# PetarKirov/Chess2RT

Hardware: AMD Instinct MI355X
Metric: Mray/s (reference-equivalent rays per second: one primary ray per sample + one shadow ray per (hit, lit light), counted as the reference casts them; ms/frame in ms_per_step) (higher is better)
Workload: dtype f64; 1 GPU; lecture5.sdl 3840x2160, 5 tap(s)/pixel (AAEnabled as shipped: reference 5-tap AA), dof off; primary_rays_per_frame=41472000, full=False

## Files before the change

### chess2rt_amd/_abi.py

```python
import ctypes as C
import os

_HERE = os.path.dirname(os.path.abspath(__file__))
_VARIANT = os.environ.get("C2RT_LIB_VARIANT", "")
LIB_PATH = os.path.join(_HERE, "libc2rt%s.so" % ("_" + _VARIANT if _VARIANT else ""))

OK, ERR_INVALID_ARG, ERR_NO_DEVICE, ERR_HIP, ERR_UNSUPPORTED, ERR_LIMIT, ERR_NO_SCENE, ERR_CANCELLED, ERR_IO, ERR_PARSE = range(10)
GEOM_PLANE, GEOM_SPHERE, GEOM_CUBE, GEOM_CSG_UNION, GEOM_CSG_INTER, GEOM_CSG_DIFF = range(6)
SHADER_LAMBERT, SHADER_PHONG = 0, 1
TEX_CHECKER, TEX_PROCEDURE2, TEX_BITMAP = 0, 1, 2
LIGHT_POINT = 0
TAPS_1, TAPS_REF5, TAPS_4 = 1, 5, 4
ABI_VERSION = 1
MAX_CSG_DEPTH = 4
MAX_CSG_HITS = 8
MAX_BATCH_FRAMES = 256
MAX_RAYS = 1 << 28
MAX_HIT_LAYERS = 16
AA_THRESHOLD_REF = 0.1

_i32p = C.POINTER(C.c_int32)
_u32p = C.POINTER(C.c_uint32)
_u64p = C.POINTER(C.c_uint64)
_f32p = C.POINTER(C.c_float)
# ... 169 lines not shown
        ("pos", C.c_double * 3),
        ("yaw", C.c_double), ("pitch", C.c_double), ("roll", C.c_double), ("fov", C.c_double),
        ("focal_plane_dist", C.c_double), ("f_number", C.c_double), ("disc_multiplier", C.c_double),
        ("dof", C.c_uint32),
        ("num_samples", C.c_uint64),
        ("stereo_separation", C.c_double),
    ]


_SCENE_P = C.POINTER(SceneDesc)
_CAM_P = C.POINTER(CameraFrame)
_OPTS_P = C.POINTER(RenderOpts)
_POSE_P = C.POINTER(ScenePose)
_VP = C.c_void_p

C2RT_SYMBOLS = {
    "c2rt_init": (C.c_int, [C.c_int, C.POINTER(_VP)]),
    "c2rt_init_multi": (C.c_int, [C.c_int, C.POINTER(C.c_int), C.POINTER(_VP)]),
    "c2rt_device_count": (C.c_int, [_VP]),
    "c2rt_scene_generation": (C.c_uint64, [_VP]),
    "c2rt_get_csg_truncations": (C.c_int, [_VP, C.POINTER(C.c_uint64)]),
    "c2rt_get_exact_redos": (C.c_int, [_VP, C.POINTER(C.c_uint64)]),
    "c2rt_get_ground_bails": (C.c_int, [_VP, C.POINTER(C.c_uint64)]),
    "c2rt_destroy": (None, [_VP]),
    "c2rt_last_error": (C.c_char_p, [_VP]),
    "c2rt_status_string": (C.c_char_p, [C.c_int]),
    "c2rt_abi_version": (C.c_uint32, []),
    "c2rt_upload_scene": (C.c_int, [_VP, _SCENE_P]),
    "c2rt_update_scene": (C.c_int, [_VP, _POSE_P, _VP]),
    "c2rt_local_rows": (C.c_uint32, [_OPTS_P]),
    "c2rt_render_frame": (C.c_int, [_VP, _CAM_P, _OPTS_P, _VP, _VP]),
    "c2rt_render_frame_device": (C.c_int, [_VP, _CAM_P, _OPTS_P, _VP, _VP]),
    "c2rt_render_frames": (C.c_int, [_VP, _CAM_P, C.c_uint32, _OPTS_P, _VP, _VP]),
    "c2rt_render_frames_device": (C.c_int, [_VP, _CAM_P, C.c_uint32, _OPTS_P, _VP, _VP]),
    "c2rt_render_frames_posed": (C.c_int, [_VP, _CAM_P, _POSE_P, C.c_uint32, _OPTS_P, _VP, _VP]),
    "c2rt_render_frames_posed_device": (C.c_int, [_VP, _CAM_P, _POSE_P, C.c_uint32, _OPTS_P, _VP, _VP]),
    "c2rt_pin_host_buffer": (C.c_int, [_VP, _VP, C.c_size_t]),
    "c2rt_unpin_host_buffer": (C.c_int, [_VP, _VP]),
    "c2rt_get_ray_stats": (C.c_int, [_VP, C.POINTER(RayStats)]),
    "c2rt_render_pixel": (C.c_int, [_VP, _CAM_P, _OPTS_P, C.c_int, C.c_int, C.POINTER(TraceResult)]),
    "c2rt_trace_rays_device": (C.c_int, [_VP, _VP, C.c_uint64, _VP, _VP, _VP]),
    "c2rt_trace_rays": (C.c_int, [_VP, _VP, C.c_uint64, _VP, _VP]),
    "c2rt_test_visibility_device": (C.c_int, [_VP, _VP, C.c_uint64, _VP, _VP]),
    "c2rt_test_visibility": (C.c_int, [_VP, _VP, C.c_uint64, _VP]),
    "c2rt_render_hits_device": (C.c_int, [_VP, _CAM_P, _OPTS_P, C.POINTER(HitPlanes), _VP]),
    "c2rt_render_hits": (C.c_int, [_VP, _CAM_P, _OPTS_P, C.POINTER(HitPlanes)]),
# ... 88 lines not shown
```

### chess2rt_amd/api.py

```python
import ctypes as C

import numpy as np

from . import _abi
from ._abi import (CameraFrame, HitPlanes, HostCamera, HostSettings, Ray, RayHit, RayStats, RenderOpts, SceneDesc, ScenePose, Segment,
                   ShadePlanes, TraceResult)

RAY_HIT_DTYPE = np.dtype({
    "names": ["closest_node", "leaf_geom", "dist", "u", "v", "p", "normal"],
    "formats": [np.int32, np.int32, np.float64, np.float64, np.float64, (np.float64, 3), (np.float64, 3)],
    "offsets": [RayHit.closest_node.offset, RayHit.leaf_geom.offset, RayHit.dist.offset, RayHit.u.offset, RayHit.v.offset,
                RayHit.p.offset, RayHit.normal.offset],
    "itemsize": C.sizeof(RayHit),
})


HIT_PLANES = {"node": (np.int32, 1), "leaf": (np.int32, 1), "dist": (np.float64, 1), "uv": (np.float64, 2),
              "p": (np.float64, 3), "normal": (np.float64, 3), "rgb": (np.float32, 3)}


def _new_hit_planes(names, rows, width):
    names = tuple(names)
    for n in names:
        if n not in HIT_PLANES:
# ... 373 lines not shown
        self._check(self._lib.c2rt_render_frames_posed_adaptive_device(self._h, arr, parr, n, C.byref(opts), float(threshold),
                                                                       C.c_void_p(out_ptr or None), C.c_void_p(mask_ptr or None), C.c_void_p(stream)))

    def rayStats(self):
        s = RayStats()
        self._check(self._lib.c2rt_get_ray_stats(self._h, C.byref(s)))
        return int(s.primary_rays), int(s.shadow_rays)

    def csgTruncations(self):
        n = C.c_uint64()
        self._check(self._lib.c2rt_get_csg_truncations(self._h, C.byref(n)))
        return int(n.value)

    def exactRedos(self):
        n = C.c_uint64()
        self._check(self._lib.c2rt_get_exact_redos(self._h, C.byref(n)))
        return int(n.value)

    def groundBails(self):
        n = C.c_uint64()
        self._check(self._lib.c2rt_get_ground_bails(self._h, C.byref(n)))
        return int(n.value)

    def renderPixel(self, cam, opts, x, y):
        r = TraceResult()
        self._check(self._lib.c2rt_render_pixel(self._h, C.byref(cam), C.byref(opts), int(x), int(y), C.byref(r)))
        return r

    def traceRays(self, rays, hits=True, colors=True):
        rays = np.ascontiguousarray(rays, dtype=np.float64)
        if rays.ndim != 2 or rays.shape[1] != 6:
            raise ValueError("rays: expected shape (n, 6), got %r" % (rays.shape,))
        n = rays.shape[0]
        rec = np.empty(n, dtype=RAY_HIT_DTYPE) if hits else None
        rgb = np.empty((n, 3), dtype=np.float32) if colors else None
        self._check(self._lib.c2rt_trace_rays(self._h, rays.ctypes.data_as(C.c_void_p), n,
                                              rec.ctypes.data_as(C.c_void_p) if hits else None,
                                              rgb.ctypes.data_as(C.c_void_p) if colors else None))
        return rec, rgb

    def traceRaysDevice(self, rays_ptr, n, hits_ptr, rgb_ptr, stream=0):
        self._check(self._lib.c2rt_trace_rays_device(self._h, C.c_void_p(rays_ptr), int(n), C.c_void_p(hits_ptr or None),
                                                     C.c_void_p(rgb_ptr or None), C.c_void_p(stream)))

    def traceRayLayers(self, rays, max_layers, hits=True, colors=True):
        rays = np.ascontiguousarray(rays, dtype=np.float64)
# ... 225 lines not shown
```

### chess2rt_amd/csrc/c2rt_api.cpp

```cpp
#include <hip/hip_runtime.h>

#include <atomic>
#include <cmath>
#include <cstdint>
#include <cstdarg>
#include <cstdio>
#include <cstdlib>
#include <cstring>
#include <memory>
#include <string>
#include <utility>
#include <vector>

#include "c2rt_query.h"
#include "scene_plan.h"

using namespace c2rt;

constexpr int kMaxChunks = 16;

constexpr int kScratchSlots = 16;
struct FrameScratch {
    const void *key = nullptr;
    bool used = false;
// ... 479 lines not shown
    }
}

const char *c2rt_last_error(const c2rt_ctx *ctx) { return ctx ? ctx->err.c_str() : "null context"; }

int c2rt_init(int device, c2rt_ctx **out)
{
    if (!out) return C2RT_ERR_INVALID_ARG;
    *out = nullptr;
    int count = 0;
    if (hipGetDeviceCount(&count) != hipSuccess || count <= 0) return C2RT_ERR_NO_DEVICE;
    if (device >= count) return C2RT_ERR_NO_DEVICE;
    if (device < 0 && hipGetDevice(&device) != hipSuccess) return C2RT_ERR_NO_DEVICE;
    c2rt_ctx *ctx = new c2rt_ctx();
    ctx->device = device;
    *out = ctx;
    HIP_TRY(ctx, hipSetDevice(device));
    HIP_TRY(ctx, hipStreamCreateWithFlags(&ctx->stream, hipStreamNonBlocking));
    HIP_TRY(ctx, hipStreamCreateWithFlags(&ctx->copy_stream, hipStreamNonBlocking));
    for (int i = 0; i < kMaxChunks; ++i) HIP_TRY(ctx, hipEventCreateWithFlags(&ctx->chunk_done[i], hipEventDisableTiming));
    HIP_TRY(ctx, hipEventCreateWithFlags(&ctx->ev_ready, hipEventDisableTiming));
    HIP_TRY(ctx, hipEventCreateWithFlags(&ctx->ev_done, hipEventDisableTiming));
    HIP_TRY(ctx, hipEventCreateWithFlags(&ctx->ev_inflight, hipEventDisableTiming));
    HIP_TRY(ctx, hipMalloc(reinterpret_cast<void **>(&ctx->counters), 5 * sizeof(unsigned long long)));
    HIP_TRY(ctx, hipMemset(ctx->counters, 0, 5 * sizeof(unsigned long long)));
    HIP_TRY(ctx, hipMalloc(reinterpret_cast<void **>(&ctx->probe), sizeof(c2rt_trace_result)));
    uint8_t lut[4097];
    build_srgb_lut(lut);
    HIP_TRY(ctx, hipMalloc(reinterpret_cast<void **>(&ctx->srgb_lut), sizeof lut));
    HIP_TRY(ctx, hipMemcpy(ctx->srgb_lut, lut, sizeof lut, hipMemcpyHostToDevice));
    return C2RT_OK;
}

int c2rt_init_multi(int device_count_or_0, const int *device_ids, c2rt_ctx **out)
{
    if (!out) return C2RT_ERR_INVALID_ARG;
    *out = nullptr;
    int visible = 0;
    if (hipGetDeviceCount(&visible) != hipSuccess || visible <= 0) return C2RT_ERR_NO_DEVICE;
    if (device_count_or_0 < 0 || device_count_or_0 > 64) return C2RT_ERR_INVALID_ARG;
    const int n = device_count_or_0 == 0 ? visible : device_count_or_0;
    std::vector<int> ids(n);
    for (int i = 0; i < n; ++i) {
        ids[i] = (device_ids && device_count_or_0 > 0) ? device_ids[i] : i;
        if (ids[i] < 0 || ids[i] >= visible) return C2RT_ERR_NO_DEVICE;
    }
    c2rt_ctx *lead = nullptr;
    int st = c2rt_init(ids[0], &lead);
// ... 573 lines not shown
    }
    if (!ctx->peers.empty()) HIP_TRY(ctx, hipSetDevice(ctx->device));
    return C2RT_OK;
}

int c2rt_get_ground_bails(c2rt_ctx *ctx, uint64_t *out)
{
    if (!ctx || !out) return C2RT_ERR_INVALID_ARG;
    HIP_TRY(ctx, hipSetDevice(ctx->device));
    HIP_TRY(ctx, hipDeviceSynchronize());
    unsigned long long h = 0;
    HIP_TRY(ctx, hipMemcpy(&h, ctx->counters + 4, sizeof h, hipMemcpyDeviceToHost));
    *out = h;
    for (c2rt_ctx *c : ctx->peers) {
        HIP_TRY(ctx, hipSetDevice(c->device));
        HIP_TRY(ctx, hipDeviceSynchronize());
        HIP_TRY(ctx, hipMemcpy(&h, c->counters + 4, sizeof h, hipMemcpyDeviceToHost));
        *out += h;
    }
    if (!ctx->peers.empty()) HIP_TRY(ctx, hipSetDevice(ctx->device));
    return C2RT_OK;
}

int c2rt_render_pixel(c2rt_ctx *ctx, const c2rt_camera_frame *cam, const c2rt_render_opts *opts, int x, int y,
                      c2rt_trace_result *out)
{
    int st = check_frame_args(ctx, cam, opts);
    if (st != C2RT_OK) return st;
    if (!out) return fail(ctx, C2RT_ERR_INVALID_ARG, "null output");
    HIP_TRY(ctx, hipSetDevice(ctx->device));
    RenderParams p;
    frame_params(ctx, cam, opts, p);
    p.n_cull = 0;
    p.ground_fast = 0;
    p.ground_certain_cq = 0;
    p.n_cull_lights = 0;
    p.csg_cap = (uint32_t)kCsgFullCap(C2RT_MAX_CSG_DEPTH);
    p.probe_x = x;
    p.probe_y = y;
    p.probe_out = ctx->probe;
    HIP_TRY(ctx, hipMemsetAsync(ctx->probe, 0, sizeof(c2rt_trace_result), ctx->stream));
    const int e = launch_probe(p, variant_of(ctx->plan, cam), ctx->stream);
    if (e != 0) return fail(ctx, C2RT_ERR_HIP, "probe kernel launch: %s", hipGetErrorString((hipError_t)e));
    HIP_TRY(ctx, hipMemcpyAsync(out, ctx->probe, sizeof *out, hipMemcpyDeviceToHost, ctx->stream));
    HIP_TRY(ctx, hipStreamSynchronize(ctx->stream));
    return C2RT_OK;
// ... 765 lines not shown
```

### chess2rt_amd/csrc/c2rt_shade_planes.hip

```cpp
#define C2RT_TRACE_EXACT_ONLY
#include "c2rt_trace_common.inc"
#include "c2rt_query.inc"

namespace c2rt {
namespace {

struct ShadeParts {
    F3 albedo, light, specular;
    uint32_t visible;
};

template <int LEVELS, bool MLC>
DEV ShadeParts shade_parts(const RenderParams &P, const Ctx &cx, const Mat &mat, D3 rd, const Surf &h, bool want_albedo, bool lit)
{
    using namespace exact;
    ShadeParts r;
    const bool phong = mat.shader_type == C2RT_SHADER_PHONG;
    const D3 N = dot(rd, h.n) < 0 ? h.n : -h.n;
    r.albedo = mkf(0, 0, 0);
    if (want_albedo) r.albedo = mat.tex_type >= 0 ? tex_color(P, mat, h.u, h.v) : mat.color;
    F3 lightContrib = mkf(P.ambient[0], P.ambient[1], P.ambient[2]);
    F3 specular = mkf(0, 0, 0);
    uint32_t word = 0;
    if (lit) {
        if constexpr (!MLC) {
            if (P.n_lights) {
                LightP L = (LightP)P.lights;
                F3 avgColor = mkf(0, 0, 0), avgSpecular = mkf(0, 0, 0);
                if (L->lit & 1u) {
                    const D3 lightPos = ld3(L->pos);
                    const D3 from = h.p + N * 1e-6;
                    double cosTheta, cosGamma;
                    F3 baseLight;
                    light_terms(cx, L, lightPos, h.p, N, rd, phong, cosTheta, baseLight, cosGamma);
                    const bool visible = test_visibility<LEVELS, 0>(cx, from, lightPos, cx.shadow_mask0, cx.shadow_ground_only);
                    if (visible) {
                        word = 1u;
                        if (cosTheta > 0) avgColor = avgColor + baseLight * (float)cosTheta;
                        if (phong & (cosGamma > 0))
                            avgSpecular = avgSpecular + baseLight * c2_pow_f32(cosGamma, mat.exponent) * mat.strength;
                    }
                }
                lightContrib = lightContrib + avgColor;
                specular = specular + avgSpecular;
            }
        } else {
            const D3 p = h.p;
            const double exponent = mat.exponent;
            const float strength = mat.strength;
            const uint32_t nl = P.n_lights;
            for (uint32_t l0 = 0; l0 < nl; l0 += 32u) {
                const uint32_t l1 = l0 + 32u < nl ? l0 + 32u : nl;
                uint32_t vis = 0;
                for (uint32_t l = l0; l < l1; ++l) {
                    LightP L = (LightP)P.lights + l;
                    if (L->lit & 1u) {
                        const D3 from = p + N * 1e-6;
                        if (test_visibility<LEVELS, 0>(cx, from, ld3(L->pos), l == 0 ? cx.shadow_mask0 : light_shadow_mask(P, cx.mask_slot, l), l == 0 && cx.shadow_ground_only))
                            vis |= 1u << (l - l0);
                    }
                }
                if (l0 == 0) word = vis;
                for (uint32_t l = l0; l < l1; ++l) {
                    LightP L = (LightP)P.lights + l;
                    F3 avgColor = mkf(0, 0, 0), avgSpecular = mkf(0, 0, 0);
                    if ((L->lit & 1u) && ((vis >> (l - l0)) & 1u)) {
                        double cosTheta, cosGamma;
                        F3 baseLight;
                        light_terms(cx, L, ld3(L->pos), p, N, rd, phong, cosTheta, baseLight, cosGamma);
                        if (cosTheta > 0) avgColor = avgColor + baseLight * (float)cosTheta;
                        if (phong & (cosGamma > 0))
                            avgSpecular = avgSpecular + baseLight * c2_pow_f32(cosGamma, exponent) * strength;
                    }
                    lightContrib = lightContrib + avgColor;
                    specular = specular + avgSpecular;
                }
            }
        }
    }
    r.light = lightContrib;
    r.specular = specular;
    r.visible = word;
    return r;
}

template <int LEVELS, bool MLC>
DEV void shade_sample(const RenderParams &P, const Ctx &cx, const c2rt_shade_planes &out, const size_t idx, D3 o, D3 d)
{
    using namespace exact;
    const bool lit = out.light || out.specular || out.visible || out.rgb;
    const bool want_albedo = out.albedo || out.rgb;
    Hit best;
// ... 80 lines not shown
```

### chess2rt_amd/csrc/c2rt_tile_mask.inc

```

DEV size_t tile_mask_slot(const RenderParams &P, uint32_t trow, uint32_t tcol)
{
    const uint32_t per_class = ((P.mask_rows + kTileH - 1) / kTileH + 7u) / 8u;
    return ((size_t)(trow & 7u) * per_class + (trow >> 3)) * (P.blocks_x * kWavesPerBlock) + tcol;
}

static_assert(kMaxCullLights <= 4, "one table word per culled light beyond the first");
DEV uint32_t light_shadow_mask(const RenderParams &P, uint32_t mask_slot, uint32_t l)
{
    if (!P.n_cull || l >= P.n_cull_lights) return 0xFFFFFFFFu;
    return ((const uint32_t C2RT_K *)P.tile_masks)[((size_t)P.mask_entries + mask_slot) * 4u + (l - 1u)];
}

DEV void tile_mask_entry(const RenderParams &P, KArgs K, const VoidCull &V, const SphereCull &S, const DarkCull *Dp, uint32_t trow, uint32_t tcol, uint32_t out[8])
{
    typedef const int C2RT_K *KInt;
    typedef const char C2RT_K *KChar;
    int tx0 = (int)(tcol * kTileW), ty0, ty1;
    {
        const uint32_t lr_first = trow * kTileH + P.mask_row0;
        uint32_t lr_last = trow * kTileH + kTileH - 1;
        if (lr_last >= P.mask_rows) lr_last = P.mask_rows - 1;
        lr_last += P.mask_row0;
        ty0 = (int)lr_first;
// ... 101 lines not shown
            const bool in_reach = fmax(fabs(fx0), fabs(fx1)) + fmax(fabs(fz0), fabs(fz1)) + fabs(gy) <= S.reach;
            for (uint32_t j = 0; j < S.n; ++j) {
                const SphereNode &sn = S.s[j];
                if (!in_reach || !((smask0 >> sn.node) & 1u) || !(sn.flags & 2u)) continue;
                if (!have_scone) { scone = shadow_cone(); have_scone = true; }
                if (cone_misses_ball(V.light0, scone, sn.c, sn.rp)) smask0 &= ~(1u << sn.node);
            }
            if (Dp && Dp->n) {
                const DarkCull &D = *Dp;
                double sdir[4][3];
                footprint_dirs(V.light0, gy, fx0, fx1, fz0, fz1, sdir);
                const bool dark_reach = fmax(fabs(fx0), fabs(fx1)) + fmax(fabs(fz0), fabs(fz1)) + fabs(gy) <= D.reach;
                for (uint32_t j = 0; j < D.n; ++j) {
                    const DarkNode &dn = D.d[j];
                    if (dn.node >= nc) continue;
                    KDbl sr = rects_s + 4 * dn.node;
                    if ((sr[1] < fx0 - padx) | (sr[0] > fx1 + padx) | (sr[3] < fz0 - padz) | (sr[2] > fz1 + padz)) continue;
                    if (tile_dark_by(V.light0, sdir, dark_reach, dn)) dark = true;
                }
            }
        }
        ground_only = (smask0 & (0xFFFFFFFFu >> (32u - nn))) == (1u << gnode);
    }
    out[0] = pmask;
    out[1] = smask0;
    out[2] = (primary_ground ? 1u : 0u) | (ground_only ? 2u : 0u) | (dark ? 4u : 0u);
    out[3] = 0;
    out[4] = out[5] = out[6] = 0xFFFFFFFFu;
    out[7] = 0;
    for (uint32_t l = 1; l < P.n_cull_lights; ++l) {
        const int *sl = P.light_side[l];
        const bool l_left = tx0 >= sl[0] && tx0 <= sl[1], l_right = sx1 >= sl[2] && sx1 <= sl[3];
        const bool l_top = ty0 >= sl[4] && ty0 <= sl[5], l_bottom = sy1 >= sl[6] && sy1 <= sl[7];
        uint32_t sm = 0xFFFFFFFFu;
        for (uint32_t n = 0; n < nc; ++n) {
            const int r0 = rects[4 * n + 0], r1 = rects[4 * n + 1], r2 = rects[4 * n + 2], r3 = rects[4 * n + 3];
            if ((l_left && r2 <= tx0) || (l_right && r0 >= sx1) || (l_top && r3 <= ty0) || (l_bottom && r1 >= sy1)) sm &= ~(1u << n);
        }
        out[3 + l] = sm;
    }
}
```

### chess2rt_amd/csrc/c2rt_trace.inc

```

DEV void len_inv(Oob &bad, double s, double &len, double &inv)
{
    if constexpr (kLean) {
        oob_note_nonneg(bad, s);
        inv_len(s, len, inv);
    } else {
        len = sqrt(s);
        inv = 1.0 / len;
    }
}
DEV void len_inv_unit(Oob &bad, double s, double &len, double &inv)
{
    if constexpr (kLean) {
        if (__all(near_one(s))) {
            unit_len(s, len, inv);
            return;
        }
    }
    len_inv(bad, s, len, inv);
}
DEV double sqrt_g(Oob &bad, double x)
{
    if constexpr (kLean) {
        oob_note(bad, x);
// ... 558 lines not shown
    }
    double rlen, rinv;
    len_inv(cx.bad, sqmag(raw), rlen, rinv);
    const D3 dir = mk(raw.x * rinv, raw.y * rinv, raw.z * rinv);
    const RayW ray = make_ray(cx.bad, from, dir);
    Hit temp;
    temp.dist = rlen;
    for (; n < nn; n = next_node(node_mask, n + 1))
        if (node_intersect<LEVELS, kBool, PO>(cx, cx.nodes + n, ray, temp)) return false;
    return true;
}


DEV F3 base_light(Oob &bad, LightP L, double r2)
{
    const float r2f = (float)r2;
    if (kLean && (L->lit & 2u)) {
        oob_note_f32(bad, r2f);
        const float rr = rcp_refined_f32(r2f);
        return mkf(div_with_f32(L->color[0], r2f, rr), div_with_f32(L->color[1], r2f, rr), div_with_f32(L->color[2], r2f, rr));
    }
    return ldf3(L->color) / r2f;
}
DEV void light_terms(const Ctx &cx, LightP L, D3 lightPos, D3 p, D3 N, D3 rd, bool phong, double &cosTheta, F3 &baseLight, double &cosGamma)
{
    const D3 lv = lightPos - p;
    const double r2 = sqmag(lv);
    double rlen, rinv;
    len_inv(cx.bad, r2, rlen, rinv);
    const D3 lightDir = mk(lv.x * rinv, lv.y * rinv, lv.z * rinv);
    cosTheta = dot(lightDir, N);
    baseLight = base_light(cx.bad, L, r2);
    cosGamma = 0;
    if (phong) {
        const D3 ml = -lightDir;
        const D3 rv = ml - N * (2 * dot(ml, N));
        double rl, ri;
        len_inv_unit(cx.bad, sqmag(rv), rl, ri);
        const D3 R = rv * ri;
        cosGamma = dot(R, -rd);
    }
}

template <int LEVELS, bool MLC, int PO>
DEV F3 shade(const RenderParams &P, const Ctx &cx, const Mat &mat, D3 rd, const Surf &h, uint32_t &shadow_rays)
{
    const bool phong = mat.shader_type == C2RT_SHADER_PHONG;
    const D3 N = dot(rd, h.n) < 0 ? h.n : -h.n;
    C2RT_REGION_BEGIN(cx, kRegTexture)
    const F3 diffuse = mat.tex_type >= 0 ? tex_color(P, mat, h.u, h.v) : mat.color;
    C2RT_REGION_END(cx, kRegTexture)
    F3 lightContrib = mkf(P.ambient[0], P.ambient[1], P.ambient[2]);
    F3 specular = mkf(0, 0, 0);
    if constexpr (!MLC) {
        if (P.n_lights) {
            LightP L = (LightP)P.lights;
            F3 avgColor = mkf(0, 0, 0), avgSpecular = mkf(0, 0, 0);
            if (L->lit & 1u) {
                const D3 lightPos = ld3(L->pos);
                shadow_rays += 1;
                const D3 from = h.p + N * 1e-6;
                double cosTheta, cosGamma;
                F3 baseLight;
                light_terms(cx, L, lightPos, h.p, N, rd, phong, cosTheta, baseLight, cosGamma);
                C2RT_REGION_BEGIN(cx, kRegShadow)
                const bool visible = test_visibility<LEVELS, PO>(cx, from, lightPos, cx.shadow_mask0, cx.shadow_ground_only);
                C2RT_REGION_END(cx, kRegShadow)
                if (visible) {
                    C2RT_REGION_BEGIN(cx, kRegLight)
                    if (cosTheta > 0) avgColor = avgColor + baseLight * (float)cosTheta;
                    if (phong & (cosGamma > 0))
                        avgSpecular = avgSpecular + baseLight * c2_pow_f32(cosGamma, mat.exponent) * mat.strength;
                    C2RT_REGION_END(cx, kRegLight)
                }
            }
            lightContrib = lightContrib + avgColor;
            specular = specular + avgSpecular;
        }
    } else {
        const D3 p = h.p;
        const double exponent = mat.exponent;
        const float strength = mat.strength;
        const uint32_t nl = P.n_lights;
        for (uint32_t l0 = 0; l0 < nl; l0 += 32u) {
            const uint32_t l1 = l0 + 32u < nl ? l0 + 32u : nl;
            uint32_t vis = 0;
            for (uint32_t l = l0; l < l1; ++l) {
                LightP L = (LightP)P.lights + l;
                if (L->lit & 1u) {
                    shadow_rays += 1;
                    const D3 from = p + N * 1e-6;
                    if (test_visibility<LEVELS, PO>(cx, from, ld3(L->pos), l == 0 ? cx.shadow_mask0 : light_shadow_mask(P, cx.mask_slot, l), l == 0 && cx.shadow_ground_only))
                        vis |= 1u << (l - l0);
                }
            }
            for (uint32_t l = l0; l < l1; ++l) {
                LightP L = (LightP)P.lights + l;
                F3 avgColor = mkf(0, 0, 0), avgSpecular = mkf(0, 0, 0);
                if ((L->lit & 1u) && ((vis >> (l - l0)) & 1u)) {
                    double cosTheta, cosGamma;
                    F3 baseLight;
                    light_terms(cx, L, ld3(L->pos), p, N, rd, phong, cosTheta, baseLight, cosGamma);
                    if (cosTheta > 0) avgColor = avgColor + baseLight * (float)cosTheta;
                    if (phong & (cosGamma > 0))
                        avgSpecular = avgSpecular + baseLight * c2_pow_f32(cosGamma, exponent) * strength;
                }
                lightContrib = lightContrib + avgColor;
                specular = specular + avgSpecular;
            }
        }
    }
    const F3 res = diffuse * lightContrib;
    return phong ? res + specular : res;
}


template <int DOF>
DEV void screen_ray(Oob &bad, const RenderParams &P, double x, double y, int offset, Rng &rng, D3 &orig, D3 &dir)
{
    const c2rt_camera_frame &cam = P.cam;
    const D3 pos = ld3(cam.pos), upLeft = ld3(cam.up_left);
    double fx, fy;
    if constexpr (kLean) {
        fx = div_with(x, cam.frame_width, P.cam_rw);
        fy = div_with(y, cam.frame_height, P.cam_rh);
// ... 326 lines not shown
                        const float b = div_with_f32(L->color[0], r2f, rcp_refined_f32(r2f));
                        const float a = 0.0f + b * cosf;
                        avgColor = mkf(a, a, a);
                    } else {
                        avgColor = avgColor + base_light(bad, L, (double)r2f) * cosf;
                    }
                }
                lightContrib = lightContrib + avgColor;
            }
            c = diffuse * lightContrib;
        }
        unsure |= u;
        accum = s == 0 ? c : accum + c;
    }
    if (ntaps > 1) tap_average(bad, accum, (float)ntaps);
    if (__ballot(unsure | oob_any(bad))) {
        if (lane == (int)__builtin_ctzll(__ballot(true))) atomicAdd(P.redo_counter + 1, 1ull);
        return kGroundBail;
    }
    store_pixel(P, (size_t)(P.frame_rows ? y : lr) * P.width + x, accum);
    return kGroundDone;
}

template <int LEVELS, int DOF, bool MLC, int PO, bool CNT>
DEV bool render_tile(const RenderParams &P, KArgs K, const uint32_t b)
{
    extern __shared__ __align__(16) char lds_all[];
    const int lane = threadIdx.x & (kWave - 1);
    const int wave = threadIdx.x / kWave;
    char *lds = lds_all + (size_t)wave * P.csg_cap * kCsgLdsPerEntry;

    const uint32_t xcd = b & 7u, j = b >> 3;
    const uint32_t groups = (P.tiles_y + 7u) / 8u;
    uint32_t grp = j / P.blocks_x + P.row_group_start;
    if (grp >= groups) grp -= groups;
    const uint32_t trow = grp * 8u + xcd, bcol = j % P.blocks_x;
    if (trow >= P.tiles_y) return false;
    const uint32_t tcol = bcol * kWavesPerBlock + wave;
#if C2RT_TILE_STATS
    const unsigned long long stamp0 = __builtin_amdgcn_s_memtime();
#endif

    uint32_t pmask = 0xFFFFFFFFu, smask0 = 0xFFFFFFFFu, mask_slot = 0;
    bool ground_only = false, primary_ground = false, dark = false;
    Oob tile_bad;
    oob_init(tile_bad);
    if constexpr (!DOF) {
        if (P.n_cull) {
            typedef uint32_t __attribute__((ext_vector_type(4))) u4_t;
            mask_slot = (uint32_t)tile_mask_slot(P, trow + (P.row_offset - P.mask_row0) / kTileH, (uint32_t)__builtin_amdgcn_readfirstlane(tcol));
            const u4_t m = ((const u4_t C2RT_K *)P.tile_masks)[mask_slot];
            pmask = m.x;
            smask0 = m.y;
            primary_ground = (m.z & 1u) != 0;
            ground_only = (m.z & 2u) != 0;
            dark = (m.z & 4u) != 0;
        }
    }

    if constexpr (kLean && LEVELS <= 1 && !DOF && !MLC && !CNT && !(PO & kSpecPlanes) && !C2RT_TILE_STATS) {
        if (P.ground_fast && (ground_only || dark)) {
            KArgs Kg = K;
            uint32_t trow_g = trow, bcol_g = bcol, dark_g = (uint32_t)__builtin_amdgcn_readfirstlane(dark && !ground_only ? 1 : 0);
            asm volatile("" : "+s"(Kg), "+s"(trow_g), "+s"(bcol_g), "+s"(dark_g));
            if (((const RenderParams *)Kg)->ground_certain_cq > 0) {
                const int gc = ground_tile_certain<PO>(*(const RenderParams *)Kg, Kg, trow_g, bcol_g, dark_g != 0);
                if (!__ballot(gc == kGroundBail)) return false;
                asm volatile("" : "+s"(Kg), "+s"(trow_g), "+s"(bcol_g), "+s"(dark_g));
            }
            const int g = ground_tile<PO>(*(const RenderParams *)Kg, Kg, trow_g, bcol_g, dark_g != 0);
            if (!__ballot(g == kGroundBail)) return g == kGroundRedo;
        }
    }

    if (P.n_nodes == 1u && P.ground_node == 0) primary_ground = true;

    const uint32_t x = tcol * kTileW + (lane % kTileW);
    const uint32_t lr0 = trow * kTileH + (lane / kTileW);
    if (x >= P.width || lr0 >= P.local_rows) return false;
    const uint32_t lr = lr0 + P.row_offset;

    uint32_t y = lr;
    if (P.strip_world > 1) {
        const uint32_t sh = P.strip_height;
        y = ((lr / sh) * P.strip_world + P.strip_rank) * sh + lr % sh;
    }

    Ctx cx;
    cx.geoms = (GeomP)P.geoms;
    cx.nodes = (NodeP)P.nodes;
    cx.n_nodes = P.n_nodes;
    cx.kargs = K;
    cx.lds = lds;
// ... 93 lines not shown
```

### chess2rt_amd/csrc/csg_void.h

```cpp
#ifndef C2RT_CSG_VOID_H
#define C2RT_CSG_VOID_H

#include <math.h>
#include <stdint.h>

#if defined(__HIPCC__)
#define C2RT_VOID_FN __host__ __device__ inline
#else
#define C2RT_VOID_FN inline
#endif

namespace c2rt {

constexpr int kMaxVoidNodes = 4;

struct VoidNode {
    double lo[3], hi[3];
    double c[3];
    double r2;
    uint32_t node;
    uint32_t flags;
};

struct VoidCull {
// ... 74 lines not shown
        const double r = sqrt(v.r2) - (t * tan_t * (1 + 1e-9) + 1e-9 * t);
        if (!(r > 0)) return false;
        const double d0 = apex[0] + u[0] * t - v.c[0], d1 = apex[1] + u[1] * t - v.c[1], d2 = apex[2] + u[2] * t - v.c[2];
        ok = ok && d0 * d0 + d1 * d1 + d2 * d2 <= r * r * (1 - 1e-12);
    }
    return ok;
}

C2RT_VOID_FN bool pyramid_void(const double apex[3], const double dir[4][3], const VoidNode &v)
{
    return pyramid_void(apex, pyramid_cone(dir), v);
}

constexpr int kMaxSphereNodes = 4;

struct SphereNode {
    double c[3];
    double rp;
    uint32_t node;
    uint32_t flags;
};

struct SphereCull {
    uint32_t n, pad;
    double reach;
    SphereNode s[kMaxSphereNodes];
};

C2RT_VOID_FN double sphere_margin(double scale, double R) { return void_margin(scale) + 1e-9 * scale * scale / R; }

C2RT_VOID_FN bool cone_misses_ball(const double apex[3], const PyramidCone &k, const double c[3], double rp)
{
    if (!k.ok) return false;
    const double w0 = c[0] - apex[0], w1 = c[1] - apex[1], w2 = c[2] - apex[2];
    const double a = w0 * k.u[0] + w1 * k.u[1] + w2 * k.u[2];
    const double e0 = w0 - a * k.u[0], e1 = w1 - a * k.u[1], e2 = w2 - a * k.u[2];
    const double lat = sqrt(e0 * e0 + e1 * e1 + e2 * e2);
    const double d = sqrt(w0 * w0 + w1 * w1 + w2 * w2);
    const double sec = sqrt(1.0 + k.tan_t * k.tan_t);
    if (!(d < 1e150) || !(rp < 1e150) || !(rp > 0) || !(sec < 1e150)) return false;
    const double need = rp * (1 + 1e-9) + 1e-9 * d;
    if (!(d > need)) return false;
    if (a + lat * k.tan_t >= 0) return lat - a * k.tan_t > need * sec;
    return true;
}

C2RT_VOID_FN void tile_corner_dirs(const double pos[3], const double ul[3], const double du[3], const double dv[3],
// ... 87 lines not shown
                                   3.3166247903554, 3.3166247903554, 3.3166247903554};
    double te0[4];
    for (int e = 0; e < 4; ++e) {
        double te1;
        if (!segment_clip_box(light, sdir[e], k.lo, k.hi, te0[e], te1)) return false;
    }
    double rel[3];
    for (int i = 0; i < 3; ++i) rel[i] = light[i] - k.c[i];
    bool dark = false;
    for (int q = 0; q < kDarkCuts; ++q) {
        const double s0 = sg[0] * w[q][0], s1 = sg[1] * w[q][1], s2 = sg[2] * w[q][2];
        const double a = s0 * rel[0] + s1 * rel[1] + s2 * rel[2] - k.r * len[q] * (1 + 1e-12);
        bool ok = true;
        for (int e = 0; e < 4; ++e) {
            const double b0 = s0 * sdir[e][0], b1 = s1 * sdir[e][1], b2 = s2 * sdir[e][2];
            const double b = b0 + b1 + b2;
            ok = ok && b < -1e-5 * (void_abs(b0) + void_abs(b1) + void_abs(b2)) && a + te0[e] * b >= 0;
        }
        dark = dark || ok;
    }
    return dark;
}

}

#endif
```

### chess2rt_amd/csrc/scene_plan.cpp

```cpp
#include "scene_plan.h"
#include "ground_certain.h"

#include <algorithm>
#include <climits>
#include <cmath>
#include <cstdarg>
#include <cstdio>
#include <cstring>
#include <utility>

namespace c2rt {
namespace {

int fail(std::string &err, int status, const char *fmt, ...)
{
    char buf[512];
    va_list ap;
    va_start(ap, fmt);
    vsnprintf(buf, sizeof buf, fmt, ap);
    va_end(ap);
    err = buf;
    return status;
}

// ... 1002 lines not shown
    if (knobs.debug_cull & 8) flags_mask = 0;
    double scale = 0;
    for (const SphereNode &seed : plan.sphere_nodes)
        scale = std::max(scale, seed.rp + std::max(std::fabs(seed.c[0]), std::max(std::fabs(seed.c[1]), std::fabs(seed.c[2]))));
    scale += std::max(std::fabs(p.cam.pos[0]), std::max(std::fabs(p.cam.pos[1]), std::fabs(p.cam.pos[2])));
    if (!plan.light_pos.empty())
        scale += std::max(std::fabs(plan.light_pos[0]), std::max(std::fabs(plan.light_pos[1]), std::fabs(plan.light_pos[2])));
    if (!std::isfinite(scale) || !(flags_mask & 3u)) return sc;
    sc.reach = scale;
    for (const SphereNode &seed : plan.sphere_nodes) {
        if (seed.node >= p.n_cull) continue;
        SphereNode s = seed;
        s.rp = seed.rp + sphere_margin(scale, seed.rp);
        if (!std::isfinite(s.rp)) continue;
        if (p.n_cull_lights == 0 || p.ground_node < 0 || plan.light_pos.empty()) s.flags &= ~2u;
        if (s.flags & 2u) {
            const double Ly = plan.light_pos[1], h = Ly - p.ground_y;
            const double tol = 1e-6 + 1e-9 * (std::fabs(Ly) + std::fabs(s.c[1]) + s.rp);
            if (!((h > 0 && s.c[1] + s.rp < Ly - tol) || (h < 0 && s.c[1] - s.rp > Ly + tol))) s.flags &= ~2u;
        }
        s.flags &= flags_mask;
        if (s.flags) sc.s[sc.n++] = s;
    }
    return sc;
}

bool dark_frame_ok(const ScenePlan &plan, const DiagKnobs &knobs, const RenderParams &p)
{
    if ((knobs.debug_cull & 32) || !plan.dark.n || p.ground_node < 0 || !p.n_cull || plan.light_pos.size() < 3) return false;
    const double h = plan.light_pos[1] - p.ground_y, eye = p.cam.pos[1] - p.ground_y;
    if (!((h > 0 && eye > 0) || (h < 0 && eye < 0))) return false;
    const double cam_mag = std::max(std::fabs(p.cam.pos[0]), std::max(std::fabs(p.cam.pos[1]), std::fabs(p.cam.pos[2])));
    return cam_mag <= plan.dark.eye_max;
}

DarkCull dark_cull_of(const ScenePlan &plan, const DiagKnobs &knobs, const RenderParams &p)
{
    return dark_frame_ok(plan, knobs, p) ? plan.dark : DarkCull{};
}

}
```

### include/c2rt.h

```cpp
#ifndef C2RT_H
#define C2RT_H

#include <stddef.h>
#include <stdint.h>

#ifdef __cplusplus
extern "C" {
#endif

#define C2RT_ABI_VERSION 1u

#define C2RT_MAX_CSG_DEPTH 4
#define C2RT_MAX_CSG_GEOMS 4096
#define C2RT_MAX_CSG_HITS 8

typedef enum c2rt_status {
    C2RT_OK = 0,
    C2RT_ERR_INVALID_ARG = 1,
    C2RT_ERR_NO_DEVICE = 2,
    C2RT_ERR_HIP = 3,
    C2RT_ERR_UNSUPPORTED = 4,
    C2RT_ERR_LIMIT = 5,
    C2RT_ERR_NO_SCENE = 6,
    C2RT_ERR_CANCELLED = 7,
// ... 163 lines not shown
                              float *out_rgb_dev, void *hip_stream);

int c2rt_render_frames(c2rt_ctx *ctx, const c2rt_camera_frame *cams,
                       uint32_t n_frames, const c2rt_render_opts *opts,
                       float *out_rgb, const volatile uint8_t *stop_flag);

int c2rt_render_frames_posed_device(c2rt_ctx *ctx, const c2rt_camera_frame *cams,
                                    const c2rt_scene_pose *poses, uint32_t n_frames,
                                    const c2rt_render_opts *opts, float *out_rgb_dev,
                                    void *hip_stream);
int c2rt_render_frames_posed(c2rt_ctx *ctx, const c2rt_camera_frame *cams,
                             const c2rt_scene_pose *poses, uint32_t n_frames,
                             const c2rt_render_opts *opts, float *out_rgb,
                             const volatile uint8_t *stop_flag);

int c2rt_get_ray_stats(c2rt_ctx *ctx, c2rt_ray_stats *out);

int c2rt_get_csg_truncations(c2rt_ctx *ctx, uint64_t *out);

int c2rt_get_exact_redos(c2rt_ctx *ctx, uint64_t *out);

int c2rt_get_ground_bails(c2rt_ctx *ctx, uint64_t *out);

int c2rt_render_pixel(c2rt_ctx *ctx, const c2rt_camera_frame *cam,
                      const c2rt_render_opts *opts, int x, int y,
                      c2rt_trace_result *out);


#define C2RT_MAX_RAYS (1u << 28)

typedef struct c2rt_ray     { double orig[3], dir[3]; } c2rt_ray;
typedef struct c2rt_segment { double from[3], to[3];  } c2rt_segment;
typedef struct c2rt_ray_hit {
    int32_t closest_node;
    int32_t leaf_geom;
    double dist, u, v;
    double p[3], normal[3];
} c2rt_ray_hit;

int c2rt_trace_rays_device(c2rt_ctx *ctx, const c2rt_ray *rays_dev, uint64_t n,
                           c2rt_ray_hit *hits_dev, float *rgb_dev, void *hip_stream);
int c2rt_trace_rays(c2rt_ctx *ctx, const c2rt_ray *rays, uint64_t n, c2rt_ray_hit *hits, float *rgb);

int c2rt_test_visibility_device(c2rt_ctx *ctx, const c2rt_segment *seg_dev, uint64_t n,
                                uint8_t *visible_dev, void *hip_stream);
int c2rt_test_visibility(c2rt_ctx *ctx, const c2rt_segment *seg, uint64_t n, uint8_t *visible);
// ... 102 lines not shown
```

Before: 143,000 Mray/s.

## Add sphere-interior tile fast path that shades a single sphere directly

```diff
diff --git a/chess2rt_amd/_abi.py b/chess2rt_amd/_abi.py
--- a/chess2rt_amd/_abi.py
+++ b/chess2rt_amd/_abi.py
@@ -215,6 +215,7 @@
     "c2rt_get_csg_truncations": (C.c_int, [_VP, C.POINTER(C.c_uint64)]),
     "c2rt_get_exact_redos": (C.c_int, [_VP, C.POINTER(C.c_uint64)]),
     "c2rt_get_ground_bails": (C.c_int, [_VP, C.POINTER(C.c_uint64)]),
+    "c2rt_get_sphere_bails": (C.c_int, [_VP, C.POINTER(C.c_uint64)]),
     "c2rt_destroy": (None, [_VP]),
     "c2rt_last_error": (C.c_char_p, [_VP]),
     "c2rt_status_string": (C.c_char_p, [C.c_int]),
diff --git a/chess2rt_amd/api.py b/chess2rt_amd/api.py
--- a/chess2rt_amd/api.py
+++ b/chess2rt_amd/api.py
@@ -419,6 +419,11 @@
         self._check(self._lib.c2rt_get_ground_bails(self._h, C.byref(n)))
         return int(n.value)
 
+    def sphereBails(self):
+        n = C.c_uint64()
+        self._check(self._lib.c2rt_get_sphere_bails(self._h, C.byref(n)))
+        return int(n.value)
+
     def renderPixel(self, cam, opts, x, y):
         r = TraceResult()
         self._check(self._lib.c2rt_render_pixel(self._h, C.byref(cam), C.byref(opts), int(x), int(y), C.byref(r)))
diff --git a/chess2rt_amd/csrc/c2rt_api.cpp b/chess2rt_amd/csrc/c2rt_api.cpp
--- a/chess2rt_amd/csrc/c2rt_api.cpp
+++ b/chess2rt_amd/csrc/c2rt_api.cpp
@@ -525,8 +525,8 @@
     HIP_TRY(ctx, hipEventCreateWithFlags(&ctx->ev_ready, hipEventDisableTiming));
     HIP_TRY(ctx, hipEventCreateWithFlags(&ctx->ev_done, hipEventDisableTiming));
     HIP_TRY(ctx, hipEventCreateWithFlags(&ctx->ev_inflight, hipEventDisableTiming));
-    HIP_TRY(ctx, hipMalloc(reinterpret_cast<void **>(&ctx->counters), 5 * sizeof(unsigned long long)));
-    HIP_TRY(ctx, hipMemset(ctx->counters, 0, 5 * sizeof(unsigned long long)));
+    HIP_TRY(ctx, hipMalloc(reinterpret_cast<void **>(&ctx->counters), 6 * sizeof(unsigned long long)));
+    HIP_TRY(ctx, hipMemset(ctx->counters, 0, 6 * sizeof(unsigned long long)));
     HIP_TRY(ctx, hipMalloc(reinterpret_cast<void **>(&ctx->probe), sizeof(c2rt_trace_result)));
     uint8_t lut[4097];
     build_srgb_lut(lut);
@@ -1146,6 +1146,24 @@
     return C2RT_OK;
 }
 
+int c2rt_get_sphere_bails(c2rt_ctx *ctx, uint64_t *out)
+{
+    if (!ctx || !out) return C2RT_ERR_INVALID_ARG;
+    HIP_TRY(ctx, hipSetDevice(ctx->device));
+    HIP_TRY(ctx, hipDeviceSynchronize());
+    unsigned long long h = 0;
+    HIP_TRY(ctx, hipMemcpy(&h, ctx->counters + 5, sizeof h, hipMemcpyDeviceToHost));
+    *out = h;
+    for (c2rt_ctx *c : ctx->peers) {
+        HIP_TRY(ctx, hipSetDevice(c->device));
+        HIP_TRY(ctx, hipDeviceSynchronize());
+        HIP_TRY(ctx, hipMemcpy(&h, c->counters + 5, sizeof h, hipMemcpyDeviceToHost));
+        *out += h;
+    }
+    if (!ctx->peers.empty()) HIP_TRY(ctx, hipSetDevice(ctx->device));
+    return C2RT_OK;
+}
+
 int c2rt_render_pixel(c2rt_ctx *ctx, const c2rt_camera_frame *cam, const c2rt_render_opts *opts, int x, int y,
                       c2rt_trace_result *out)
 {
diff --git a/chess2rt_amd/csrc/c2rt_shade_planes.hip b/chess2rt_amd/csrc/c2rt_shade_planes.hip
--- a/chess2rt_amd/csrc/c2rt_shade_planes.hip
+++ b/chess2rt_amd/csrc/c2rt_shade_planes.hip
@@ -32,7 +32,7 @@
                     const D3 from = h.p + N * 1e-6;
                     double cosTheta, cosGamma;
                     F3 baseLight;
-                    light_terms(cx, L, lightPos, h.p, N, rd, phong, cosTheta, baseLight, cosGamma);
+                    light_terms(cx.bad, L, lightPos, h.p, N, rd, phong, cosTheta, baseLight, cosGamma);
                     const bool visible = test_visibility<LEVELS, 0>(cx, from, lightPos, cx.shadow_mask0, cx.shadow_ground_only);
                     if (visible) {
                         word = 1u;
@@ -67,7 +67,7 @@
                     if ((L->lit & 1u) && ((vis >> (l - l0)) & 1u)) {
                         double cosTheta, cosGamma;
                         F3 baseLight;
-                        light_terms(cx, L, ld3(L->pos), p, N, rd, phong, cosTheta, baseLight, cosGamma);
+                        light_terms(cx.bad, L, ld3(L->pos), p, N, rd, phong, cosTheta, baseLight, cosGamma);
                         if (cosTheta > 0) avgColor = avgColor + baseLight * (float)cosTheta;
                         if (phong & (cosGamma > 0))
                             avgSpecular = avgSpecular + baseLight * c2_pow_f32(cosGamma, exponent) * strength;
diff --git a/chess2rt_amd/csrc/c2rt_tile_mask.inc b/chess2rt_amd/csrc/c2rt_tile_mask.inc
--- a/chess2rt_amd/csrc/c2rt_tile_mask.inc
+++ b/chess2rt_amd/csrc/c2rt_tile_mask.inc
@@ -147,9 +147,24 @@
         }
         ground_only = (smask0 & (0xFFFFFFFFu >> (32u - nn))) == (1u << gnode);
     }
+    bool interior = false;
+    if (__builtin_expect(S.interior != 0u, 0) && nn >= 1u && nn <= 32u) {
+        const uint32_t live = pmask & (0xFFFFFFFFu >> (32u - nn));
+        const uint32_t gbit = gnode >= 0 ? 1u << gnode : 0u;
+        const uint32_t rest = live & ~gbit;
+        if ((live & gbit) == gbit && rest && !(rest & (rest - 1u)) && (rest & S.interior)) {
+            for (uint32_t j = 0; j < S.n; ++j) {
+                const SphereNode &sn = S.s[j];
+                if ((1u << sn.node) != rest) continue;
+                if (!have_pcone) { pcone = primary_cone(); have_pcone = true; }
+                const double R = ((NodeP)P.nodes)[sn.node].g.p[3];
+                interior = sphere_interior_tile(P.cam.pos, pcone, S, j, R, V, smask0, nn, gnode, P.ground_y, P.n_lights != 0u);
+            }
+        }
+    }
     out[0] = pmask;
     out[1] = smask0;
-    out[2] = (primary_ground ? 1u : 0u) | (ground_only ? 2u : 0u) | (dark ? 4u : 0u);
+    out[2] = (primary_ground ? 1u : 0u) | (ground_only ? 2u : 0u) | (dark ? 4u : 0u) | (interior ? 8u : 0u);
     out[3] = 0;
     out[4] = out[5] = out[6] = 0xFFFFFFFFu;
     out[7] = 0;
diff --git a/chess2rt_amd/csrc/c2rt_trace.inc b/chess2rt_amd/csrc/c2rt_trace.inc
--- a/chess2rt_amd/csrc/c2rt_trace.inc
+++ b/chess2rt_amd/csrc/c2rt_trace.inc
@@ -604,21 +604,21 @@
     }
     return ldf3(L->color) / r2f;
 }
-DEV void light_terms(const Ctx &cx, LightP L, D3 lightPos, D3 p, D3 N, D3 rd, bool phong, double &cosTheta, F3 &baseLight, double &cosGamma)
+DEV void light_terms(Oob &bad, LightP L, D3 lightPos, D3 p, D3 N, D3 rd, bool phong, double &cosTheta, F3 &baseLight, double &cosGamma)
 {
     const D3 lv = lightPos - p;
     const double r2 = sqmag(lv);
     double rlen, rinv;
-    len_inv(cx.bad, r2, rlen, rinv);
+    len_inv(bad, r2, rlen, rinv);
     const D3 lightDir = mk(lv.x * rinv, lv.y * rinv, lv.z * rinv);
     cosTheta = dot(lightDir, N);
-    baseLight = base_light(cx.bad, L, r2);
+    baseLight = base_light(bad, L, r2);
     cosGamma = 0;
     if (phong) {
         const D3 ml = -lightDir;
         const D3 rv = ml - N * (2 * dot(ml, N));
         double rl, ri;
-        len_inv_unit(cx.bad, sqmag(rv), rl, ri);
+        len_inv_unit(bad, sqmag(rv), rl, ri);
         const D3 R = rv * ri;
         cosGamma = dot(R, -rd);
     }
@@ -644,7 +644,7 @@
                 const D3 from = h.p + N * 1e-6;
                 double cosTheta, cosGamma;
                 F3 baseLight;
-                light_terms(cx, L, lightPos, h.p, N, rd, phong, cosTheta, baseLight, cosGamma);
+                light_terms(cx.bad, L, lightPos, h.p, N, rd, phong, cosTheta, baseLight, cosGamma);
                 C2RT_REGION_BEGIN(cx, kRegShadow)
                 const bool visible = test_visibility<LEVELS, PO>(cx, from, lightPos, cx.shadow_mask0, cx.shadow_ground_only);
                 C2RT_REGION_END(cx, kRegShadow)
@@ -682,7 +682,7 @@
                 if ((L->lit & 1u) && ((vis >> (l - l0)) & 1u)) {
                     double cosTheta, cosGamma;
                     F3 baseLight;
-                    light_terms(cx, L, ld3(L->pos), p, N, rd, phong, cosTheta, baseLight, cosGamma);
+                    light_terms(cx.bad, L, ld3(L->pos), p, N, rd, phong, cosTheta, baseLight, cosGamma);
                     if (cosTheta > 0) avgColor = avgColor + baseLight * (float)cosTheta;
                     if (phong & (cosGamma > 0))
                         avgSpecular = avgSpecular + baseLight * c2_pow_f32(cosGamma, exponent) * strength;
@@ -1055,6 +1055,121 @@
     return kGroundDone;
 }
 
+template <int PO>
+DEV int sphere_tile(const RenderParams &P, KArgs K, const uint32_t trow, const uint32_t bcol, const uint32_t node)
+{
+    static_assert(!(PO & kSpecPlanes), "the planes-only instances have no mask table");
+    const int lane = threadIdx.x & (kWave - 1);
+    const int wave = threadIdx.x / kWave;
+    const uint32_t tcol = bcol * kWavesPerBlock + wave;
+    const uint32_t x = tcol * kTileW + (lane % kTileW);
+    const uint32_t lr0 = trow * kTileH + (lane / kTileW);
+    if (x >= P.width || lr0 >= P.local_rows) return kGroundDone;
+    const uint32_t lr = lr0 + P.row_offset;
+    const uint32_t y = frame_row(P, lr);
+    const uint32_t ntaps = P.taps;
+
+    Oob bad;
+    oob_init(bad);
+    bool missed = false;
+    F3 accum = mkf(0, 0, 0);
+#pragma unroll 1
+    for (uint32_t s = 0; s < ntaps; ++s) {
+        KArgs Kt = K;
+        asm volatile("" : "+s"(Kt));
+        const RenderParams &Pt = *(const RenderParams *)Kt;
+        Rng rng = {0u, 0, 0};
+        D3 o, raw;
+        screen_ray<0>(bad, Pt, (double)x + k_aa_x[s], (double)y + k_aa_y[s], 0, rng, o, raw);
+        const D3 d = normalized(bad, raw);
+        NodeP N = (NodeP)Pt.nodes + node;
+        GeomP G = &N->g;
+        const bool has_off = !(N->flags & kNodeZeroOffset);
+        const RayW ray = make_ray(bad, o, d);
+        Hit h;
+        {
+            ORay rc;
+            rc.o = ray.o;
+            if (has_off) rc.o = rc.o - ld3(N->off);
+            rc.d = ray.dn;
+            rc.A = ray.A;
+            prep_dir(rc, kPrepA);
+            h.dist = 1e99 * ray.len;
+            h.p = ray.o;
+            missed |= !sphere_intersect<kFull>(bad, G, N->geom, rc, h, false);
+        }
+        Mat mat;
+        load_mat(N, mat);
+        const D3 pc = h.p - ld3(G->p);
+        D3 n = normalized(bad, pc);
+        F3 diffuse = mat.color;
+        if (mat.tex_type >= 0) {
+            double u, v;
+            const double sc = (double)__uint_as_float(mat.td[2]);
+            sphere_uv(pc.x, pc.z, pc.y / G->p[3], UVWant{kUVBitmap, sc}, u, v);
+            u *= sc;
+            v *= sc;
+            u = u - floor(u);
+            v = v - floor(v);
+            const uint32_t w = mat.td[0], hgt = mat.td[1];
+            diffuse = bitmap_filtered_uniform(Pt.texels, mat.td[4], w, hgt, (float)u * (float)w, (float)v * (float)hgt);
+        }
+        {
+            double len, inv;
+            len_inv_unit(bad, sqmag(n), len, inv);
+            n = n * inv;
+        }
+        D3 p = h.p;
+        if (has_off) p = p + ld3(N->off);
+        const bool phong = mat.shader_type == C2RT_SHADER_PHONG;
+        const D3 Nf = dot(d, n) < 0 ? n : -n;
+        F3 lightContrib = mkf(Pt.ambient[0], Pt.ambient[1], Pt.ambient[2]);
+        F3 specular = mkf(0, 0, 0);
+        if (Pt.n_lights) {
+            LightP L = (LightP)Pt.lights;
+            F3 avgColor = mkf(0, 0, 0), avgSpecular = mkf(0, 0, 0);
+            if (L->lit & 1u) {
+                const D3 lightPos = ld3(L->pos);
+                const D3 from = p + Nf * 1e-6;
+                double cosTheta, cosGamma;
+                F3 baseLight;
+                light_terms(bad, L, lightPos, p, Nf, d, phong, cosTheta, baseLight, cosGamma);
+                const D3 sraw = lightPos - from;
+                double rlen, rinv;
+                len_inv(bad, sqmag(sraw), rlen, rinv);
+                const RayW sray = make_ray(bad, from, mk(sraw.x * rinv, sraw.y * rinv, sraw.z * rinv));
+                ORay rc;
+                rc.o = sray.o;
+                if (has_off) rc.o = rc.o - ld3(N->off);
+                rc.d = sray.dn;
+                rc.A = sray.A;
+                prep_dir(rc, kPrepA);
+                Hit t;
+                t.dist = rlen * sray.len;
+                const bool visible = !sphere_intersect<kBool>(bad, G, N->geom, rc, t, false);
+                if (visible) {
+                    if (cosTheta > 0) avgColor = avgColor + baseLight * (float)cosTheta;
+                    if (phong & (cosGamma > 0))
+                        avgSpecular = avgSpecular + baseLight * c2_pow_f32(cosGamma, mat.exponent) * mat.strength;
+                }
+            }
+            lightContrib = lightContrib + avgColor;
+            specular = specular + avgSpecular;
+        }
+        const F3 res = diffuse * lightContrib;
+        const F3 c = phong ? res + specular : res;
+        accum = s == 0 ? c : accum + c;
+    }
+    if (ntaps > 1) accum = accum / (float)ntaps;
+    if (__ballot(missed)) {
+        if (lane == (int)__builtin_ctzll(__ballot(true))) atomicAdd(P.redo_counter + 2, 1ull);
+        return kGroundBail;
+    }
+    if (__ballot(oob_any(bad))) return kGroundRedo;
+    store_pixel(P, (size_t)(P.frame_rows ? y : lr) * P.width + x, accum);
+    return kGroundDone;
+}
+
 template <int LEVELS, int DOF, bool MLC, int PO, bool CNT>
 DEV bool render_tile(const RenderParams &P, KArgs K, const uint32_t b)
 {
@@ -1075,7 +1190,7 @@
 #endif
 
     uint32_t pmask = 0xFFFFFFFFu, smask0 = 0xFFFFFFFFu, mask_slot = 0;
-    bool ground_only = false, primary_ground = false, dark = false;
+    bool ground_only = false, primary_ground = false, dark = false, interior = false;
     Oob tile_bad;
     oob_init(tile_bad);
     if constexpr (!DOF) {
@@ -1088,6 +1203,7 @@
             primary_ground = (m.z & 1u) != 0;
             ground_only = (m.z & 2u) != 0;
             dark = (m.z & 4u) != 0;
+            interior = (m.z & 8u) != 0;
         }
     }
 
@@ -1102,6 +1218,15 @@
                 asm volatile("" : "+s"(Kg), "+s"(trow_g), "+s"(bcol_g), "+s"(dark_g));
             }
             const int g = ground_tile<PO>(*(const RenderParams *)Kg, Kg, trow_g, bcol_g, dark_g != 0);
+            if (!__ballot(g == kGroundBail)) return g == kGroundRedo;
+        }
+        if (__builtin_expect(interior, 0)) {
+            uint32_t rest = pmask & (0xFFFFFFFFu >> (32u - P.n_nodes));
+            if (P.ground_node >= 0) rest &= ~(1u << P.ground_node);
+            KArgs Ks = K;
+            uint32_t trow_s = trow, bcol_s = bcol, node_s = (uint32_t)__builtin_amdgcn_readfirstlane((int)__builtin_ctz(rest | 0x80000000u));
+            asm volatile("" : "+s"(Ks), "+s"(trow_s), "+s"(bcol_s), "+s"(node_s));
+            const int g = sphere_tile<PO>(*(const RenderParams *)Ks, Ks, trow_s, bcol_s, node_s);
             if (!__ballot(g == kGroundBail)) return g == kGroundRedo;
         }
     }
diff --git a/chess2rt_amd/csrc/csg_void.h b/chess2rt_amd/csrc/csg_void.h
--- a/chess2rt_amd/csrc/csg_void.h
+++ b/chess2rt_amd/csrc/csg_void.h
@@ -120,7 +120,8 @@
 };
 
 struct SphereCull {
-    uint32_t n, pad;
+    uint32_t n;
+    uint32_t interior;
     double reach;
     SphereNode s[kMaxSphereNodes];
 };
@@ -254,6 +255,135 @@
     return dark;
 }
 
+
+C2RT_VOID_FN bool cone_inside_ball(const double apex[3], const PyramidCone &k, const double c[3], double R, double m, double &t_lo,
+                                   double &t_hi)
+{
+    t_lo = t_hi = 0;
+    if (!k.ok) return false;
+    const double w0 = c[0] - apex[0], w1 = c[1] - apex[1], w2 = c[2] - apex[2];
+    const double a = w0 * k.u[0] + w1 * k.u[1] + w2 * k.u[2];
+    const double e0 = w0 - a * k.u[0], e1 = w1 - a * k.u[1], e2 = w2 - a * k.u[2];
+    const double lat = sqrt(e0 * e0 + e1 * e1 + e2 * e2);
+    const double d = sqrt(w0 * w0 + w1 * w1 + w2 * w2);
+    const double sec = sqrt(1.0 + k.tan_t * k.tan_t);
+    if (!(d < 1e150) || !(R < 1e150) || !(R > 0) || !(m > 0) || !(m < R) || !(sec < 1e150) || !(a > 0)) return false;
+    if (!(d >= (R + m) * (1 + 1e-9))) return false;
+    const double inv_d = 1.0 / d, ct = 1.0 / sec;
+    const double sp = lat * inv_d, cp = a * inv_d, st = k.tan_t * ct;
+    const double s_hi = sp * ct + cp * st, c_hi = cp * ct - sp * st;
+    if (!(c_hi > 1e-9)) return false;
+    if (!(d * s_hi * (1 + 1e-9) + 1e-9 * d <= R - m)) return false;
+    double s_lo = sp * ct - cp * st, c_lo = cp * ct + sp * st;
+    if (!(s_lo > 0)) { s_lo = 0; c_lo = 1; }
+    t_lo = d * c_lo - sqrt(R * R - d * d * s_lo * s_lo);
+    t_hi = d * c_hi - sqrt(R * R - d * d * s_hi * s_hi);
+    return t_lo > 0 && t_hi >= t_lo && t_hi < 1e150;
+}
+
+struct ShadowCone {
+    double u[3];
+    double tan_t, sec;
+    bool ok;
+};
+
+C2RT_VOID_FN bool patch_shadow_cone(const double apex[3], const PyramidCone &k, double t_lo, double t_hi, double m, const double light[3],
+                                    double q[3], double &rho, ShadowCone &sc)
+{
+    const double tm = 0.5 * (t_lo + t_hi);
+    rho = (0.5 * (t_hi - t_lo) + t_hi * k.tan_t) * (1 + 1e-9) + 2 * m + 1e-9 * t_hi;
+    double v[3], D2 = 0;
+    for (int i = 0; i < 3; ++i) {
+        q[i] = apex[i] + tm * k.u[i];
+        v[i] = q[i] - light[i];
+        D2 += v[i] * v[i];
+    }
+    const double D = sqrt(D2);
+    sc.ok = false;
+    if (!(D < 1e150) || !(rho < 1e150) || !(D > 2 * rho)) return false;
+    const double inv_D = 1.0 / D, inv_h = 1.0 / sqrt(D2 - rho * rho);
+    for (int i = 0; i < 3; ++i) sc.u[i] = v[i] * inv_D;
+    sc.tan_t = rho * inv_h * (1 + 1e-9);
+    sc.sec = D * inv_h * (1 + 1e-9);
+    sc.ok = sc.tan_t < 1e150 && sc.sec < 1e150;
+    return sc.ok;
+}
+
+C2RT_VOID_FN bool shadow_cone_misses_ball(const double apex[3], const ShadowCone &k, const double c[3], double rp)
+{
+    if (!k.ok) return false;
+    const double w0 = c[0] - apex[0], w1 = c[1] - apex[1], w2 = c[2] - apex[2];
+    const double a = w0 * k.u[0] + w1 * k.u[1] + w2 * k.u[2];
+    const double e0 = w0 - a * k.u[0], e1 = w1 - a * k.u[1], e2 = w2 - a * k.u[2];
+    const double lat2 = e0 * e0 + e1 * e1 + e2 * e2, d2 = w0 * w0 + w1 * w1 + w2 * w2;
+    const double d1 = void_abs(w0) + void_abs(w1) + void_abs(w2);
+    if (!(d1 < 1e150) || !(rp < 1e150) || !(rp > 0)) return false;
+    const double need = rp * (1 + 1e-9) + 1e-9 * d1;
+    if (!(d2 > need * need * (1 + 1e-9))) return false;
+    if (a >= 0 || lat2 * k.tan_t * k.tan_t >= a * a) {
+        const double x = (a * k.tan_t + need * k.sec) * (1 + 1e-9);
+        return !(x > 0) || lat2 > x * x * (1 + 1e-9);
+    }
+    return true;
+}
+
+C2RT_VOID_FN void box_ball(const VoidNode &v, double m, double c[3], double &rp)
+{
+    double r2 = 0;
+    for (int i = 0; i < 3; ++i) {
+        c[i] = 0.5 * (v.lo[i] + v.hi[i]);
+        const double h = 0.5 * (v.hi[i] - v.lo[i]);
+        r2 += h * h;
+    }
+    rp = sqrt(r2) * (1 + 1e-9) + m;
+}
+
+C2RT_VOID_FN bool sphere_interior_rest(const double eye[3], const PyramidCone &k, const SphereCull &S, uint32_t self, double m, double t_lo,
+                                       double t_hi, const VoidCull &V, uint32_t smask0, uint32_t n_nodes, int ground_node,
+                                       double ground_y, bool has_light)
+{
+    const SphereNode &sn = S.s[self];
+    const double tol = 1e-6 + 1e-9 * (void_abs(ground_y) + void_abs(sn.c[1]) + sn.rp + void_abs(eye[1]));
+    if (ground_node >= 0 && !(eye[1] > ground_y + tol && sn.c[1] - sn.rp > ground_y + tol)) return false;
+    if (!has_light) return true;
+    const double *L = V.light0;
+    double q[3], rho;
+    ShadowCone sc;
+    if (!patch_shadow_cone(eye, k, t_lo, t_hi, m, L, q, rho, sc)) return false;
+    const double ltol = 1e-6 + 1e-9 * (void_abs(L[1]) + void_abs(q[1]) + rho + void_abs(ground_y));
+    if (ground_node >= 0 && !(L[1] > ground_y + ltol)) return false;
+    uint32_t others = smask0 & (n_nodes >= 32u ? 0xFFFFFFFFu : ((1u << n_nodes) - 1u)) & ~(1u << sn.node);
+    if (ground_node >= 0) others &= ~(1u << ground_node);
+    if (!others) return true;
+    if (!(q[1] + rho < L[1] - ltol)) return false;
+    for (uint32_t j = 0; j < S.n; ++j) {
+        const SphereNode &o = S.s[j];
+        if (j == self || !((others >> o.node) & 1u)) continue;
+        if (!(o.flags & 2u) || !shadow_cone_misses_ball(L, sc, o.c, o.rp)) return false;
+        others &= ~(1u << o.node);
+    }
+    for (uint32_t j = 0; j < V.n; ++j) {
+        const VoidNode &o = V.v[j];
+        if (!((others >> o.node) & 1u)) continue;
+        double bc[3], brp;
+        box_ball(o, m, bc, brp);
+        if (!(o.flags & 2u) || !shadow_cone_misses_ball(L, sc, bc, brp)) return false;
+        others &= ~(1u << o.node);
+    }
+    return others == 0u;
+}
+
+C2RT_VOID_FN bool sphere_interior_tile(const double eye[3], const PyramidCone &k, const SphereCull &S, uint32_t self, double R,
+                                       const VoidCull &V, uint32_t smask0, uint32_t n_nodes, int ground_node, double ground_y,
+                                       bool has_light)
+{
+    const SphereNode &sn = S.s[self];
+    const double m = sn.rp - R;
+    double t_lo, t_hi;
+    if (!cone_inside_ball(eye, k, sn.c, R, m, t_lo, t_hi)) return false;
+    return sphere_interior_rest(eye, k, S, self, m, t_lo, t_hi, V, smask0, n_nodes, ground_node, ground_y, has_light);
+}
+
 }
 
 #endif
diff --git a/chess2rt_amd/csrc/scene_plan.cpp b/chess2rt_amd/csrc/scene_plan.cpp
--- a/chess2rt_amd/csrc/scene_plan.cpp
+++ b/chess2rt_amd/csrc/scene_plan.cpp
@@ -1048,6 +1048,25 @@
         s.flags &= flags_mask;
         if (s.flags) sc.s[sc.n++] = s;
     }
+    constexpr uint64_t kSphereTileMinSamples = 6000000;
+    const uint64_t samples = (uint64_t)p.width * p.height * p.taps / (p.strip_world > 1 ? p.strip_world : 1u);
+    if (p.n_cull && plan.n_lights <= 1 && plan.csg_levels <= 1 && !p.cam.dof && p.cam.stereo_separation == 0 && !p.ray_counters &&
+        !(knobs.debug_cull & 128) &&
+        (samples >= kSphereTileMinSamples || (knobs.debug_cull & 256))) {
+        for (uint32_t j = 0; j < sc.n; ++j) {
+            const uint32_t n = sc.s[j].node;
+            if (n >= plan.nodes.size() || n >= 32u) continue;
+            const DevMat &m = plan.nodes[n].mat;
+            if (m.shader_type != C2RT_SHADER_LAMBERT && m.shader_type != C2RT_SHADER_PHONG) continue;
+            bool tex_ok = m.tex_type < 0;
+            if (m.tex_type == C2RT_TEX_BITMAP) {
+                const uint64_t w = m.texdata[0], h = m.texdata[1];
+                const uint64_t offset = (uint64_t)m.texdata[4] | ((uint64_t)m.texdata[5] << 32);
+                tex_ok = w < (1ull << 24) && h < (1ull << 24) && offset <= (1ull << 28) && w * h <= (1ull << 28) - offset;
+            }
+            if (tex_ok) sc.interior |= 1u << n;
+        }
+    }
     return sc;
 }
 
diff --git a/include/c2rt.h b/include/c2rt.h
--- a/include/c2rt.h
+++ b/include/c2rt.h
@@ -209,6 +209,8 @@
 
 int c2rt_get_ground_bails(c2rt_ctx *ctx, uint64_t *out);
 
+int c2rt_get_sphere_bails(c2rt_ctx *ctx, uint64_t *out);
+
 int c2rt_render_pixel(c2rt_ctx *ctx, const c2rt_camera_frame *cam,
                       const c2rt_render_opts *opts, int x, int y,
                       c2rt_trace_result *out);
```

After: 149,300 Mray/s, median of 6. 1.04x the previous value.
